# lRomul/sensorium

Hardware: AMD Instinct MI355X
Metric: training clips/sec/GPU (DwiseNeuro fwd+bwd, B=32 T=32 36x64) at 1/2/4/8 GPUs (higher is better)
Workload: dtype bf16

## Files before the change

### sensorium_amd/csrc/dwn_gemm_kd.hip

```cpp
#include "dwn_internal.h"
#include <type_traits>

#ifndef KD_FRG
#define KD_FRG 2
#endif
#ifndef KD_FRG256
#define KD_FRG256 1
#endif
#ifndef KD_WIDE
#define KD_WIDE 1
#endif
#ifndef KD_MINW128
#define KD_MINW128 3
#endif
typedef __attribute__((ext_vector_type(8))) short kd_bf16x8_t;
typedef __attribute__((ext_vector_type(4))) float kd_f32x4_t;

struct KdArgs {
    const bf16_t* A; i64 lda;
    const bf16_t* A2; i64 a2_ld; int K1;
    const bf16_t* B; i64 ldb;
    bf16_t* C; i64 ldc;
    int M, N, K;
    const float* bias;
    const float* gate; int gate_ld, rows_per_sample;
    double* stats; int stat_nchan;
    int ntm, ntn;
};

static __device__ __forceinline__ void kd_lds_barrier() {
    asm volatile("s_waitcnt lgkmcnt(0)" ::: "memory");
    __builtin_amdgcn_s_barrier();
    asm volatile("" ::: "memory");
}

template <int BN, int RT, bool GATE, bool CAT>
__global__ __launch_bounds__(256, BN * RT >= 512 ? 2 : KD_MINW128) void gemm_kd_kernel(const KdArgs g) {
    constexpr int BM = 64 * RT;
    constexpr int NJ = BN / 16;
    constexpr int NCH = BN * 4 / 256;
    constexpr int STG = BN * 64;
    constexpr int CROW = BN * 2 + 16;
    constexpr int CPR = BN / 8;
    constexpr int NIT = 64 * CPR / 256;
    constexpr int FRG = BN == 256 ? KD_FRG256 : KD_FRG;
    extern __shared__ __attribute__((aligned(16))) unsigned char kd_smem[];
    unsigned char* const sB = kd_smem;
    unsigned char* const sC = kd_smem + 2 * STG;
    float* const lred = reinterpret_cast<float*>(sC + 64 * CROW);
    float* const sgate = lred + 2 * BN;

    const int tid = threadIdx.x;
    const int wave = tid >> 6, lane = tid & 63, lr = lane & 15, lg = lane >> 4;
    const int t = (int)(blockIdx.x >> 3) + (int)(blockIdx.x & 7) * (int)(gridDim.x >> 3);
    const int nt = t % g.ntn, mt = t / g.ntn;
    if (mt >= g.ntm) { DET_EXIT(); return; }
    const int m0 = mt * BM, n0 = nt * BN;
    const int nk = g.K >> 5;

    const bf16_t* pa[RT];
    [[maybe_unused]] const bf16_t* pa2[RT];
#pragma unroll
    for (int i = 0; i < RT; ++i) {
        int m = m0 + 16 * RT * wave + 16 * i + lr;
        m = m < g.M ? m : g.M - 1;
        pa[i] = g.A + (i64)m * g.lda + 8 * lg;
        if constexpr (CAT) pa2[i] = g.A2 + (i64)m * g.a2_ld + 8 * lg;
    }
    uint4 ar[4][RT];
    auto load_a = [&](int ks, uint4 (&dst)[RT]) {
        ks = ks < nk ? ks : nk - 1;
        const int k = ks << 5;
#pragma unroll
        for (int i = 0; i < RT; ++i) {
            const bf16_t* src = pa[i] + k;
            if constexpr (CAT) src = k >= g.K1 ? pa2[i] + (k - g.K1) : src;
            dst[i] = *reinterpret_cast<const uint4*>(src);
        }
    };
    const bf16_t* pb[NCH];
    unsigned sboff[NCH];
#pragma unroll
    for (int i = 0; i < NCH; ++i) {
        const int c = tid + 256 * i, n = c >> 2, kc = c & 3;
        pb[i] = g.B + (i64)(n0 + n) * g.ldb + 8 * kc;
        sboff[i] = (unsigned)(n * 64 + ((kc ^ ((0 - (n >> 2)) & 3)) * 16));
    }
    uint4 bs[2][NCH];
    auto load_b = [&](int ks, uint4 (&dst)[NCH]) {
        ks = ks < nk ? ks : nk - 1;
#pragma unroll
        for (int i = 0; i < NCH; ++i) dst[i] = *reinterpret_cast<const uint4*>(pb[i] + (ks << 5));
    };
    auto store_b = [&](const int stage, const uint4 (&src)[NCH]) {
#pragma unroll
        for (int i = 0; i < NCH; ++i) *reinterpret_cast<uint4*>(sB + stage * STG + sboff[i]) = make_uint4(src[i].x, src[i].y, src[i].z, src[i].w);
    };

    kd_f32x4_t acc[RT][NJ];
#pragma unroll
    for (int i = 0; i < RT; ++i)
#pragma unroll
        for (int j = 0; j < NJ; ++j) acc[i][j] = kd_f32x4_t{0.f, 0.f, 0.f, 0.f};

#pragma unroll
    for (int u = 0; u < 4; ++u) load_a(u, ar[u]);
    load_b(0, bs[0]);
    load_b(1, bs[1]);
    if constexpr (GATE) {
        const float* grow = g.gate + (i64)(m0 / g.rows_per_sample) * g.gate_ld;
        for (int k = tid * 4; k < g.K; k += 1024) *reinterpret_cast<float4*>(sgate + k) = *reinterpret_cast<const float4*>(grow + k);
    }
    store_b(0, bs[0]);
    load_b(2, bs[0]);
    kd_lds_barrier();

    const unsigned char* const fb = sB + lr * 64 + ((lg ^ ((0 - (lr >> 2)) & 3)) * 16);
    auto step = [&](auto uc, const int ks) {
            constexpr int u = decltype(uc)::value;
            {
                constexpr int sb = (u + 1) & 1;
                const int kb = (ks + 3 < nk ? ks + 3 : nk - 1) << 5;
#pragma unroll
                for (int i = 0; i < NCH; ++i) {
                    *reinterpret_cast<uint4*>(sB + sb * STG + sboff[i]) = make_uint4(bs[sb][i].x, bs[sb][i].y, bs[sb][i].z, bs[sb][i].w);
                    bs[sb][i] = *reinterpret_cast<const uint4*>(pb[i] + kb);
                }
            }
            uint4 af[RT];
#pragma unroll
            for (int i = 0; i < RT; ++i) af[i] = ar[u][i];
            if constexpr (GATE) {
                const float4 g0 = *reinterpret_cast<const float4*>(sgate + (ks << 5) + 8 * lg);
                const float4 g1 = *reinterpret_cast<const float4*>(sgate + (ks << 5) + 8 * lg + 4);
                const float gv[8] = {g0.x, g0.y, g0.z, g0.w, g1.x, g1.y, g1.z, g1.w};
#pragma unroll
                for (int i = 0; i < RT; ++i) {
                    float v[8];
                    unpack16<bf16_t>(af[i], v);
#pragma unroll
                    for (int e = 0; e < 8; ++e) v[e] *= gv[e];
                    af[i] = pack16<bf16_t>(v);
                }
            }
            const unsigned char* const st = fb + (u & 1) * STG;
#pragma unroll
            for (int j0 = 0; j0 < NJ; j0 += FRG) {
                uint4 wf[FRG];
#pragma unroll
                for (int j = 0; j < FRG; ++j) wf[j] = *reinterpret_cast<const uint4*>(st + (j0 + j) * 1024);
                if constexpr (FRG > 1) __builtin_amdgcn_sched_barrier(0);
#pragma unroll
                for (int j = 0; j < FRG; ++j)
#pragma unroll
                    for (int i = 0; i < RT; ++i)
                        acc[i][j0 + j] = __builtin_amdgcn_mfma_f32_16x16x32_bf16(__builtin_bit_cast(kd_bf16x8_t, wf[j]), __builtin_bit_cast(kd_bf16x8_t, af[i]),
                                                                                 acc[i][j0 + j], 0, 0, 0);
            }
            if constexpr (u & 1) { load_a(ks + 3, ar[u - 1]); load_a(ks + 4, ar[u]); }
            kd_lds_barrier();
    };
    for (int ks0 = 0; ks0 < nk; ks0 += 4) {
        step(std::integral_constant<int, 0>{}, ks0);
        step(std::integral_constant<int, 1>{}, ks0 + 1);
        step(std::integral_constant<int, 2>{}, ks0 + 2);
        step(std::integral_constant<int, 3>{}, ks0 + 3);
    }

    const int ch = tid % CPR;
    float st0[8], st1[8];
#pragma unroll
    for (int e = 0; e < 8; ++e) { st0[e] = 0.f; st1[e] = 0.f; }
#pragma unroll
    for (int p = 0; p < BM / 64; ++p) {
        if (16 * RT * wave / 64 == p) {
#pragma unroll
            for (int i = 0; i < RT; ++i) {
                const int row = (16 * RT * wave) % 64 + 16 * i + lr;
#pragma unroll
                for (int j = 0; j < NJ; ++j) {
                    const int col = 16 * j + 4 * lg;
                    kd_f32x4_t v = acc[i][j];
                    if (g.bias) {
                        const float4 bv = *reinterpret_cast<const float4*>(g.bias + n0 + col);
                        v[0] += bv.x; v[1] += bv.y; v[2] += bv.z; v[3] += bv.w;
                    }
                    *reinterpret_cast<uint2*>(sC + row * CROW + col * 2) = make_uint2(pk_bf16(v[0], v[1]), pk_bf16(v[2], v[3]));
                }
            }
        }
        kd_lds_barrier();
#pragma unroll
        for (int it = 0; it < NIT; ++it) {
            const int row = tid / CPR + it * (256 / CPR);
            const int m = m0 + 64 * p + row;
            const uint4 raw = *reinterpret_cast<const uint4*>(sC + row * CROW + ch * 16);
            if (m < g.M) {
                *reinterpret_cast<uint4*>(g.C + (i64)m * g.ldc + n0 + ch * 8) = raw;
                float v[8];
                unpack16<bf16_t>(raw, v);
#pragma unroll
                for (int e = 0; e < 8; ++e) { st0[e] += v[e]; st1[e] = fmaf(v[e], v[e], st1[e]); }
            }
        }
        kd_lds_barrier();
    }
    if (g.stats) {
        for (int i = tid; i < 2 * BN; i += 256) lred[i] = 0.f;
        __syncthreads();
        DET_WAVES_BEGIN
#pragma unroll
        for (int e = 0; e < 8; ++e) {
            atomicAdd(&lred[ch * 8 + e], st0[e]);
            atomicAdd(&lred[BN + ch * 8 + e], st1[e]);
        }
        DET_WAVES_END
        __syncthreads();
        DET_ENTER();
        for (int i = tid; i < 2 * BN; i += 256)
            stat_add(g.stats, (int)(blockIdx.x % DWN_NREP), g.stat_nchan, i / BN, n0 + i % BN, lred[i]);
    }
    DET_EXIT();
}

static bool kd_args_ok(const GemmNN& g, int dtype) {
    if (dtype != DWN_BF16 || g.groups != 1 || g.b_sample_stride || g.M < 1) return false;
    if (g.epi == EPI_STORE) {
        if (g.a_kind != LD_PLAIN && g.a_kind != LD_GATE) return false;
        if (g.a2) return false;
    } else if (g.epi == EPI_STORE_CAT) {
        if (g.a_kind != LD_PLAIN || !g.a2 || !g.bias || g.K1 <= 0 || g.K1 % 32 || g.a2_ld % 8 || ((size_t)g.a2 & 15) || ((size_t)g.bias & 15)) return false;
    } else {
        return false;
    }
    if (g.a_kind == LD_GATE && (!g.a.gate || g.a.rows_per_sample <= 0 || g.a.rows_per_sample % 128 || g.a.gate_ld % 4 || ((size_t)g.a.gate & 15) || g.K > 4096))
        return false;
    if (g.K % 128 || g.N % 128 || g.a.ld % 8 || g.ldb % 8 || g.ldc % 8) return false;
    if (((size_t)g.a.p | (size_t)g.b | (size_t)g.c) & 15) return false;
    return true;
}

bool gemm_nn_kd_eligible(const GemmNN& g, int dtype) {
    if (g.variant == DWN_NN_TILE128 || g.variant == DWN_NN_XL128 || g.variant == DWN_NN_XL256) return false;
    if (!kd_args_ok(g, dtype)) return false;
    if (g.variant == DWN_NN_KD) return true;
    return g.K >= 512 && g.M >= 8192 && (g.N == 256 || (g.N == 128 && g.a_kind == LD_GATE));
}

template <int BN, int RT, bool GATE, bool CAT>
static int launch_kd_t(const KdArgs& a, hipStream_t s) {
    const size_t smem = 2 * (size_t)BN * 64 + 64 * ((size_t)BN * 2 + 16) + 2 * (size_t)BN * 4 + (GATE ? (size_t)a.K * 4 : 0);
    if (smem > 48 * 1024) {
        hipError_t e = hipFuncSetAttribute(reinterpret_cast<const void*>(gemm_kd_kernel<BN, RT, GATE, CAT>), hipFuncAttributeMaxDynamicSharedMemorySize, (int)smem);
        if (e != hipSuccess) return dwn_set_error((int)e, hipGetErrorString(e));
    }
    const unsigned tiles = (unsigned)a.ntm * (unsigned)a.ntn;
    const unsigned grid = (tiles + 7u) & ~7u;
    hipLaunchKernelGGL((gemm_kd_kernel<BN, RT, GATE, CAT>), dim3(grid), dim3(256), smem, s, a);
    DWN_CHECK_LAUNCH();
    return 0;
}

int launch_gemm_nn_kd(const GemmNN& g, hipStream_t s) {
    KdArgs a;
    a.A = reinterpret_cast<const bf16_t*>(g.a.p); a.lda = g.a.ld;
    const bool cat = g.epi == EPI_STORE_CAT;
    a.A2 = cat ? reinterpret_cast<const bf16_t*>(g.a2) : nullptr; a.a2_ld = cat ? g.a2_ld : 0; a.K1 = cat ? g.K1 : g.K;
    a.B = reinterpret_cast<const bf16_t*>(g.b); a.ldb = g.ldb;
    a.C = reinterpret_cast<bf16_t*>(g.c); a.ldc = g.ldc;
    a.M = g.M; a.N = g.N; a.K = g.K;
    a.bias = cat ? g.bias : nullptr;
    const bool gate = g.a_kind == LD_GATE;
    a.gate = gate ? g.a.gate : nullptr; a.gate_ld = gate ? g.a.gate_ld : 0; a.rows_per_sample = gate ? g.a.rows_per_sample : 1;
    a.stats = g.stats; a.stat_nchan = g.stat_nchan;
    const int ntm128 = (g.M + 127) / 128;
    const bool wide = KD_WIDE && g.N % 256 == 0 && (i64)ntm128 * (g.N / 256) >= 512;
    a.ntm = ntm128;
    a.ntn = wide ? g.N / 256 : g.N / 128;
    if (wide) {
        if (gate) return launch_kd_t<256, 2, true, false>(a, s);
        return cat ? launch_kd_t<256, 2, false, true>(a, s) : launch_kd_t<256, 2, false, false>(a, s);
    }
    if (gate) return launch_kd_t<128, 2, true, false>(a, s);
    return cat ? launch_kd_t<128, 2, false, true>(a, s) : launch_kd_t<128, 2, false, false>(a, s);
}
```

Baseline: 1472.

## Add 160-row by 256-column GEMM tile variant for better CU fill on mid-size shapes

Adds a new tile configuration for the KD bf16 GEMM: 10 waves, one row-tile per wave (160 rows) by 256 columns. It uses a deeper 8-stage A register ring and 512-thread B staging. The launcher picks this variant for N%256 shapes that would otherwise fall back to 128x128 tiles, when a cost model shows better per-CU work balance (wave quantization over 256 CUs). This trades higher registers per block and occupancy of 1 for fewer, larger tiles and less B reload. The epilogue and stats paths are guarded so only the first 256 threads do output IO.

```diff
diff --git a/sensorium_amd/csrc/dwn_gemm_kd.hip b/sensorium_amd/csrc/dwn_gemm_kd.hip
--- a/sensorium_amd/csrc/dwn_gemm_kd.hip
+++ b/sensorium_amd/csrc/dwn_gemm_kd.hip
@@ -13,6 +13,19 @@
 #ifndef KD_MINW128
 #define KD_MINW128 3
 #endif
+#ifndef KD_FILL_ROWS
+#define KD_FILL_ROWS 160
+#endif
+#ifndef KD_FILL_ST
+#define KD_FILL_ST 512
+#endif
+#ifndef KD_FILL_RING
+#define KD_FILL_RING 8
+#endif
+#define KD_FILL_NW (KD_FILL_ROWS ? KD_FILL_ROWS / 16 : 5)
+#define KD_FILL_WPC (KD_FILL_ROWS == 160 ? 1 : 2)
+static_assert(KD_FILL_ROWS == 0 || KD_FILL_ROWS == 80 || KD_FILL_ROWS == 160, "KD_FILL_ROWS: 0, 80 or 160");
+static_assert((KD_FILL_ST == 256 || KD_FILL_ST == 512) && (KD_FILL_RING == 4 || KD_FILL_RING == 8), "KD_FILL_ST: 256 or 512; KD_FILL_RING: 4 or 8");
 typedef __attribute__((ext_vector_type(8))) short kd_bf16x8_t;
 typedef __attribute__((ext_vector_type(4))) float kd_f32x4_t;
 
@@ -34,11 +47,14 @@
     asm volatile("" ::: "memory");
 }
 
-template <int BN, int RT, bool GATE, bool CAT>
-__global__ __launch_bounds__(256, BN * RT >= 512 ? 2 : KD_MINW128) void gemm_kd_kernel(const KdArgs g) {
-    constexpr int BM = 64 * RT;
+template <int BN, int RT, bool GATE, bool CAT, int NW = 4>
+__global__ __launch_bounds__(64 * NW, NW > 5 ? 1 : (BN * RT >= 512 || NW == 5) ? 2 : KD_MINW128) void gemm_kd_kernel(const KdArgs g) {
+    constexpr int NT = 64 * NW;
+    constexpr int BM = 16 * RT * NW;
+    constexpr int NP = (BM + 63) / 64;
     constexpr int NJ = BN / 16;
-    constexpr int NCH = BN * 4 / 256;
+    constexpr int ST = NW >= 8 ? KD_FILL_ST : 256;
+    constexpr int NCH = BN * 4 / ST;
     constexpr int STG = BN * 64;
     constexpr int CROW = BN * 2 + 16;
     constexpr int CPR = BN / 8;
@@ -52,6 +68,8 @@
 
     const int tid = threadIdx.x;
     const int wave = tid >> 6, lane = tid & 63, lr = lane & 15, lg = lane >> 4;
+    const bool io = NW == 4 || tid < 256;
+    const bool stg = NW == 4 || tid < ST;
     const int t = (int)(blockIdx.x >> 3) + (int)(blockIdx.x & 7) * (int)(gridDim.x >> 3);
     const int nt = t % g.ntn, mt = t / g.ntn;
     if (mt >= g.ntm) { DET_EXIT(); return; }
@@ -67,7 +85,8 @@
         pa[i] = g.A + (i64)m * g.lda + 8 * lg;
         if constexpr (CAT) pa2[i] = g.A2 + (i64)m * g.a2_ld + 8 * lg;
     }
-    uint4 ar[4][RT];
+    constexpr int RD = NW >= 8 ? KD_FILL_RING : 4;
+    uint4 ar[RD][RT];
     auto load_a = [&](int ks, uint4 (&dst)[RT]) {
         ks = ks < nk ? ks : nk - 1;
         const int k = ks << 5;
@@ -82,19 +101,21 @@
     unsigned sboff[NCH];
 #pragma unroll
     for (int i = 0; i < NCH; ++i) {
-        const int c = tid + 256 * i, n = c >> 2, kc = c & 3;
+        const int c = tid % ST + ST * i, n = c >> 2, kc = c & 3;
         pb[i] = g.B + (i64)(n0 + n) * g.ldb + 8 * kc;
         sboff[i] = (unsigned)(n * 64 + ((kc ^ ((0 - (n >> 2)) & 3)) * 16));
     }
+    auto pbi = [&](int i) { return RT == 1 ? pb[0] + (i64)i * (ST / 4) * g.ldb : pb[i]; };
+    auto sbo = [&](int i) { return RT == 1 ? sboff[0] + (unsigned)(ST * 16 * i) : sboff[i]; };
     uint4 bs[2][NCH];
     auto load_b = [&](int ks, uint4 (&dst)[NCH]) {
         ks = ks < nk ? ks : nk - 1;
 #pragma unroll
-        for (int i = 0; i < NCH; ++i) dst[i] = *reinterpret_cast<const uint4*>(pb[i] + (ks << 5));
+        for (int i = 0; i < NCH; ++i) dst[i] = *reinterpret_cast<const uint4*>(pbi(i) + (ks << 5));
     };
     auto store_b = [&](const int stage, const uint4 (&src)[NCH]) {
 #pragma unroll
-        for (int i = 0; i < NCH; ++i) *reinterpret_cast<uint4*>(sB + stage * STG + sboff[i]) = make_uint4(src[i].x, src[i].y, src[i].z, src[i].w);
+        for (int i = 0; i < NCH; ++i) *reinterpret_cast<uint4*>(sB + stage * STG + sbo(i)) = make_uint4(src[i].x, src[i].y, src[i].z, src[i].w);
     };
 
     kd_f32x4_t acc[RT][NJ];
@@ -104,27 +125,25 @@
         for (int j = 0; j < NJ; ++j) acc[i][j] = kd_f32x4_t{0.f, 0.f, 0.f, 0.f};
 
 #pragma unroll
-    for (int u = 0; u < 4; ++u) load_a(u, ar[u]);
-    load_b(0, bs[0]);
-    load_b(1, bs[1]);
+    for (int u = 0; u < RD; ++u) load_a(u, ar[u]);
+    if (stg) { load_b(0, bs[0]); load_b(1, bs[1]); }
     if constexpr (GATE) {
         const float* grow = g.gate + (i64)(m0 / g.rows_per_sample) * g.gate_ld;
-        for (int k = tid * 4; k < g.K; k += 1024) *reinterpret_cast<float4*>(sgate + k) = *reinterpret_cast<const float4*>(grow + k);
-    }
-    store_b(0, bs[0]);
-    load_b(2, bs[0]);
+        for (int k = tid * 4; k < g.K; k += 4 * NT) *reinterpret_cast<float4*>(sgate + k) = *reinterpret_cast<const float4*>(grow + k);
+    }
+    if (stg) { store_b(0, bs[0]); load_b(2, bs[0]); }
     kd_lds_barrier();
 
     const unsigned char* const fb = sB + lr * 64 + ((lg ^ ((0 - (lr >> 2)) & 3)) * 16);
     auto step = [&](auto uc, const int ks) {
             constexpr int u = decltype(uc)::value;
-            {
+            if (stg) {
                 constexpr int sb = (u + 1) & 1;
                 const int kb = (ks + 3 < nk ? ks + 3 : nk - 1) << 5;
 #pragma unroll
                 for (int i = 0; i < NCH; ++i) {
-                    *reinterpret_cast<uint4*>(sB + sb * STG + sboff[i]) = make_uint4(bs[sb][i].x, bs[sb][i].y, bs[sb][i].z, bs[sb][i].w);
-                    bs[sb][i] = *reinterpret_cast<const uint4*>(pb[i] + kb);
+                    *reinterpret_cast<uint4*>(sB + sb * STG + sbo(i)) = make_uint4(bs[sb][i].x, bs[sb][i].y, bs[sb][i].z, bs[sb][i].w);
+                    bs[sb][i] = *reinterpret_cast<const uint4*>(pbi(i) + kb);
                 }
             }
             uint4 af[RT];
@@ -157,14 +176,21 @@
                         acc[i][j0 + j] = __builtin_amdgcn_mfma_f32_16x16x32_bf16(__builtin_bit_cast(kd_bf16x8_t, wf[j]), __builtin_bit_cast(kd_bf16x8_t, af[i]),
                                                                                  acc[i][j0 + j], 0, 0, 0);
             }
-            if constexpr (u & 1) { load_a(ks + 3, ar[u - 1]); load_a(ks + 4, ar[u]); }
+            if constexpr (u & 1) { load_a(ks + RD - 1, ar[u - 1]); load_a(ks + RD, ar[u]); }
             kd_lds_barrier();
     };
-    for (int ks0 = 0; ks0 < nk; ks0 += 4) {
+    for (int ks0 = 0; ks0 < nk; ks0 += RD) {
         step(std::integral_constant<int, 0>{}, ks0);
         step(std::integral_constant<int, 1>{}, ks0 + 1);
         step(std::integral_constant<int, 2>{}, ks0 + 2);
         step(std::integral_constant<int, 3>{}, ks0 + 3);
+        if constexpr (RD == 8) {
+            if (ks0 + 4 >= nk) break;
+            step(std::integral_constant<int, 4>{}, ks0 + 4);
+            step(std::integral_constant<int, 5>{}, ks0 + 5);
+            step(std::integral_constant<int, 6>{}, ks0 + 6);
+            step(std::integral_constant<int, 7>{}, ks0 + 7);
+        }
     }
 
     const int ch = tid % CPR;
@@ -172,7 +198,7 @@
 #pragma unroll
     for (int e = 0; e < 8; ++e) { st0[e] = 0.f; st1[e] = 0.f; }
 #pragma unroll
-    for (int p = 0; p < BM / 64; ++p) {
+    for (int p = 0; p < NP; ++p) {
         if (16 * RT * wave / 64 == p) {
 #pragma unroll
             for (int i = 0; i < RT; ++i) {
@@ -192,10 +218,10 @@
         kd_lds_barrier();
 #pragma unroll
         for (int it = 0; it < NIT; ++it) {
-            const int row = tid / CPR + it * (256 / CPR);
+            const int row = (tid & 255) / CPR + it * (256 / CPR);
             const int m = m0 + 64 * p + row;
             const uint4 raw = *reinterpret_cast<const uint4*>(sC + row * CROW + ch * 16);
-            if (m < g.M) {
+            if (io && 64 * p + row < BM && m < g.M) {
                 *reinterpret_cast<uint4*>(g.C + (i64)m * g.ldc + n0 + ch * 8) = raw;
                 float v[8];
                 unpack16<bf16_t>(raw, v);
@@ -206,18 +232,20 @@
         kd_lds_barrier();
     }
     if (g.stats) {
-        for (int i = tid; i < 2 * BN; i += 256) lred[i] = 0.f;
+        for (int i = tid; i < 2 * BN; i += NT) lred[i] = 0.f;
         __syncthreads();
         DET_WAVES_BEGIN
-#pragma unroll
-        for (int e = 0; e < 8; ++e) {
-            atomicAdd(&lred[ch * 8 + e], st0[e]);
-            atomicAdd(&lred[BN + ch * 8 + e], st1[e]);
+        if (io) {
+#pragma unroll
+            for (int e = 0; e < 8; ++e) {
+                atomicAdd(&lred[ch * 8 + e], st0[e]);
+                atomicAdd(&lred[BN + ch * 8 + e], st1[e]);
+            }
         }
         DET_WAVES_END
         __syncthreads();
         DET_ENTER();
-        for (int i = tid; i < 2 * BN; i += 256)
+        for (int i = tid; i < 2 * BN; i += NT)
             stat_add(g.stats, (int)(blockIdx.x % DWN_NREP), g.stat_nchan, i / BN, n0 + i % BN, lred[i]);
     }
     DET_EXIT();
@@ -247,16 +275,16 @@
     return g.K >= 512 && g.M >= 8192 && (g.N == 256 || (g.N == 128 && g.a_kind == LD_GATE));
 }
 
-template <int BN, int RT, bool GATE, bool CAT>
+template <int BN, int RT, bool GATE, bool CAT, int NW = 4>
 static int launch_kd_t(const KdArgs& a, hipStream_t s) {
     const size_t smem = 2 * (size_t)BN * 64 + 64 * ((size_t)BN * 2 + 16) + 2 * (size_t)BN * 4 + (GATE ? (size_t)a.K * 4 : 0);
     if (smem > 48 * 1024) {
-        hipError_t e = hipFuncSetAttribute(reinterpret_cast<const void*>(gemm_kd_kernel<BN, RT, GATE, CAT>), hipFuncAttributeMaxDynamicSharedMemorySize, (int)smem);
+        hipError_t e = hipFuncSetAttribute(reinterpret_cast<const void*>(gemm_kd_kernel<BN, RT, GATE, CAT, NW>), hipFuncAttributeMaxDynamicSharedMemorySize, (int)smem);
         if (e != hipSuccess) return dwn_set_error((int)e, hipGetErrorString(e));
     }
     const unsigned tiles = (unsigned)a.ntm * (unsigned)a.ntn;
     const unsigned grid = (tiles + 7u) & ~7u;
-    hipLaunchKernelGGL((gemm_kd_kernel<BN, RT, GATE, CAT>), dim3(grid), dim3(256), smem, s, a);
+    hipLaunchKernelGGL((gemm_kd_kernel<BN, RT, GATE, CAT, NW>), dim3(grid), dim3(64 * NW), smem, s, a);
     DWN_CHECK_LAUNCH();
     return 0;
 }
@@ -275,6 +303,17 @@
     a.stats = g.stats; a.stat_nchan = g.stat_nchan;
     const int ntm128 = (g.M + 127) / 128;
     const bool wide = KD_WIDE && g.N % 256 == 0 && (i64)ntm128 * (g.N / 256) >= 512;
+    constexpr int rows = KD_FILL_ROWS ? KD_FILL_ROWS : 1;
+    if (KD_FILL_ROWS && KD_WIDE && !wide && g.N % 256 == 0 && (!gate || g.a.rows_per_sample % rows == 0)) {
+        const i64 tf = (i64)((g.M + rows - 1) / rows) * (g.N / 256), t128 = (i64)ntm128 * (g.N / 128);
+        const i64 per_cu_f = (tf + 256 * KD_FILL_WPC - 1) / (256 * KD_FILL_WPC) * KD_FILL_WPC, per_cu_128 = (t128 + 255) / 256;
+        if (tf >= 256 && per_cu_f * (rows + 256) < per_cu_128 * (128 + 128)) {
+            a.ntm = (g.M + rows - 1) / rows;
+            a.ntn = g.N / 256;
+            if (gate) return launch_kd_t<256, 1, true, false, KD_FILL_NW>(a, s);
+            return cat ? launch_kd_t<256, 1, false, true, KD_FILL_NW>(a, s) : launch_kd_t<256, 1, false, false, KD_FILL_NW>(a, s);
+        }
+    }
     a.ntm = ntm128;
     a.ntn = wide ? g.N / 256 : g.N / 128;
     if (wide) {
```

Result: no change. 1477 (median of 6 runs) (+0.3%).
